# GATB/dsk

Measured on AMD Instinct MI355X. Metric: distinct k-mers counted/sec (whole node), k=31, higher is better.
Workload: dtype u64

## Files before the change

dsk_amd/csrc/dskgpu.hip:

```cpp
#include <algorithm>
#include <cstdio>
#include <cstring>
#include <cstdlib>
#include <cmath>
#include <string>
#include <vector>

#include <thread>
#include <system_error>
#include "engine.h"
#include "kernels.h"
#include "superkmer.h"
#include "rawparse.h"

#include <rocprim/device/device_radix_sort.hpp>

#define DSKGPU_VERSION "dskgpu 0.1 (gfx950)"

namespace {

thread_local std::string g_create_err;

__global__ __launch_bounds__(1024) void k_place_probe(unsigned long long* __restrict__ out, unsigned long long n) {
    const unsigned long long per_block = n / gridDim.x, per_stream = per_block / 512;
// ... 59 lines not shown
__global__ __launch_bounds__(256) void k_setup_pass(u32* __restrict__ sc, ScalarSet h, u64* __restrict__ ghist, u32 nh, u64* __restrict__ gstats, u32 nstats,
                                                    u32* __restrict__ zero, u64 nzero) {
    const u32 t = blockIdx.x * 256 + threadIdx.x;
    if (t < SC_COUNT) sc[t] = h.v[t];
    if (t < nstats) gstats[t] = 0ull;
    for (u32 i = t; i < nh; i += gridDim.x * 256) ghist[i] = 0ull;
    for (u64 i = t; i < nzero; i += (u64)gridDim.x * 256) zero[i] = 0u;
}
}

namespace {

#define LAND_BYTES (64u << 10)
void* landing(dskgpu_ctx* ctx, size_t bytes) {
    if (bytes > LAND_BYTES) return nullptr;
    if (!ctx->land && hipHostMalloc(reinterpret_cast<void**>(&ctx->land), LAND_BYTES, hipHostMallocDefault) != hipSuccess) { ctx->land = nullptr; (void)hipGetLastError(); }
    return ctx->land;
}

bool sentinel_is_a_kmer(int W, unsigned k) {
    u64 v[4] = {0, 0, 0, 0};
    if (W == 1) v[0] = kunmix(~0ull);
    else if (W == 2) { KN<2> x; x.w[0] = x.w[1] = ~0ull; kunmixN(x); v[0] = x.w[0]; v[1] = x.w[1]; }
    else { KN<4> x; for (int i = 0; i < 4; ++i) x.w[i] = ~0ull; kunmixN(x); for (int i = 0; i < 4; ++i) v[i] = x.w[i]; }
    auto base = [&](const u64* a, unsigned i) { return (unsigned)((a[i >> 5] >> (2 * (i & 31))) & 3u); };
    for (unsigned i = k; i < 128; ++i) if (base(v, i)) return false;
    u64 r[4] = {0, 0, 0, 0};
    for (unsigned i = 0; i < k; ++i) { const unsigned c = base(v, i) ^ 2u, j = k - 1 - i; r[j >> 5] |= (u64)c << (2 * (j & 31)); }
    for (int x = 3; x >= 0; --x) if (v[x] != r[x]) return v[x] < r[x];
    return true;
}


int run_encode(dskgpu_ctx* ctx, const uint8_t* d_bytes, u64 n, u64* nwords_out) {
    const u64 nwords = (n + 31) / 32;
    ctx->enc_fresh = false;
    CK(ctx->packed.ensure((nwords + 1) * 8));
    CK(ctx->inval.ensure((nwords + 1) * 4));
    if (const int rc = encode_into(ctx, d_bytes, n, ctx->packed.as<u64>(), ctx->inval.as<u32>())) return rc;
    *nwords_out = nwords;
    return DSKGPU_OK;
}

int encode_current(dskgpu_ctx* ctx, u64* nwords_out) {
    if (ctx->enc_keep) { *nwords_out = (ctx->n_bytes + 31) / 32; ctx->enc_fresh = false; return DSKGPU_OK; }
    if (!ctx->d_reads && ctx->n_bytes) return fail(ctx, DSKGPU_E_STATE, "the reads were released (dskgpu_encode_reads) and their 2-bit form has been overwritten: set the reads again");
    return run_encode(ctx, ctx->d_reads, ctx->n_bytes, nwords_out);
}

}

int encode_into(dskgpu_ctx* ctx, const uint8_t* d_bytes, u64 n, u64* packed, u32* inval) {
    const u64 nwords = (n + 31) / 32;
    if (!nwords) return DSKGPU_OK;
    const u64 nb = (nwords + 255) / 256;
    const unsigned grid = (unsigned)std::min<u64>(nb, (u64)ctx->num_cu * 16);
    if ((reinterpret_cast<uintptr_t>(d_bytes) & 15) == 0)
        hipLaunchKernelGGL(k_encode<true>, dim3(grid), dim3(256), 0, ctx->stream, d_bytes, n, packed, inval, nwords);
    else
        hipLaunchKernelGGL(k_encode<false>, dim3(grid), dim3(256), 0, ctx->stream, d_bytes, n, packed, inval, nwords);
    CKL("k_encode");
    return DSKGPU_OK;
}

int run_scan(dskgpu_ctx* ctx, u32* a, const u32* d_len, u64 max_len) {
    const u64 nb = std::max<u64>(1, (max_len + SCAN_BLK - 1) / SCAN_BLK);
    CK(ctx->sums.ensure((nb + 1) * 4));
    hipLaunchKernelGGL(k_scan_reduce, dim3((unsigned)nb), dim3(SCAN_NT), 0, ctx->stream, a, d_len, ctx->sums.as<u32>());
    hipLaunchKernelGGL(k_scan_sums, dim3(1), dim3(1024), 0, ctx->stream, ctx->sums.as<u32>(), d_len, a);
    hipLaunchKernelGGL(k_scan_apply, dim3((unsigned)nb), dim3(SCAN_NT), 0, ctx->stream, a, d_len, ctx->sums.as<u32>());
    CKL("k_scan");
    return DSKGPU_OK;
}

int allow_big_lds(dskgpu_ctx* ctx, const void* fn, int bytes) {
    for (const void* f : ctx->big_lds_fns) if (f == fn) return DSKGPU_OK;
    CK(hipFuncSetAttribute(fn, hipFuncAttributeMaxDynamicSharedMemorySize, bytes));
    ctx->big_lds_fns.push_back(fn);
    return DSKGPU_OK;
}

namespace {

size_t scatter_lds(int W, u32 P, bool opt = false) { return (size_t)SC_NT * (16 / W) * 8 * W + (size_t)P * (opt ? 20 : 16) + 4 + 17 * 4 + 16 + (opt ? 8 + L0_MAX_PASSES * 8 : 0); }

template <int W, int SRC, int MODE>
int launch_hist_m(dskgpu_ctx* ctx, const typename KeyT<W>::T* keys, const ChunkDesc* descs, const u32* d_nch,
                  u64 max_chunks, u32* matrix, DigitSpec ds, u32 P) {
    const unsigned grid = (unsigned)std::max<u64>(1, std::min<u64>(max_chunks, (u64)ctx->num_cu));
    hipLaunchKernelGGL((k_hist<W, SRC, MODE>), dim3(grid), dim3(SC_NT), 0, ctx->stream, ctx->packed.as<u64>(),
                       ctx->inval.as<u32>(), keys, descs, d_nch, matrix, (int)ctx->cfg.kmer_size, ds, P);
    CKL("k_hist");
    return DSKGPU_OK;
// ... 1029 lines not shown
    CK(ctx->l0buf.ensure(tot * sp.R * 8 + 64));
    CK(ctx->sk_lay.ensure(SK_MAX_OWNERS * 12));
    CK(hipMemcpyAsync(ctx->sk_lay.p, obase, sizeof obase, hipMemcpyHostToDevice, ctx->stream));
    CK(hipMemcpyAsync(ctx->sk_lay.as<u64>() + SK_MAX_OWNERS, osl, sizeof osl, hipMemcpyHostToDevice, ctx->stream));
    sp.olo = olo; sp.ohi = ohi; sp.obase = ctx->sk_lay.as<unsigned long long>(); sp.oslice = reinterpret_cast<const u32*>(ctx->sk_lay.as<u64>() + SK_MAX_OWNERS);
    sp.c0 = 0; sp.c0g = 0; sp.clen = (u32)rl.nch; sp.rbase = 0; sp.slice = 0;
    u32* sc = ctx->scalars.as<u32>();
    CK(hipMemsetAsync(ctx->sk_sent.p, 0, SK_MAX_OWNERS * 8, ctx->stream));
    CK(hipMemsetAsync(sc + SC_OVF1, 0, 4, ctx->stream));
#define SK_CALL(K_, M_) hipLaunchKernelGGL((k_sk_scatter<true, K_, M_>), dim3(sp.nchunks), dim3(SK_NT), 0, ctx->stream, ctx->packed.as<u64>(), ctx->inval.as<u32>(), sp, \
                                          (const unsigned long long*)nullptr, ctx->l0buf.as<u64>(), sc + SC_OVF1, ctx->sk_sent.as<unsigned long long>())
    SK_DISPATCH(ctx, sp, SK_CALL);
#undef SK_CALL
    CKL("k_sk_scatter(passes)");
    ctx->mark("level0");
    CK(hipMemcpyAsync(&ctx->h_ovf1, sc + SC_OVF1, 4, hipMemcpyDeviceToHost, ctx->stream));
    CK(hipMemcpyAsync(ctx->h_sk_sent, ctx->sk_sent.p, SK_MAX_OWNERS * 8, hipMemcpyDeviceToHost, ctx->stream));
    CK(hipStreamSynchronize(ctx->stream));
    if (ctx->tune.verbose) fprintf(stderr, "[dskgpu] level 0 (records): passes %u..%u of %u materialised, %.2f GB%s\n", olo, ohi - 1, rl.G, (double)tot * sp.R * 8e-9,
                                   ctx->h_ovf1 ? " -- a slice overflowed: starting over on the key-array path" : "");
    return ctx->h_ovf1 ? REC_L0_NO : DSKGPU_OK;
}

template <int W>
int run_pipeline(dskgpu_ctx* ctx, bool from_reads, const typename KeyT<W>::T* d_keys_in, u64 nkeys_in) {
    typedef typename KeyT<W>::T Key;
    ctx->drop_result();
    ctx->sink = dskgpu_ctx::RowSink{};
    if (from_reads) { ctx->st_names.clear(); ctx->st_ms.clear(); }
    ctx->marks.clear(); ctx->ev_used = 0;
    const u64 n_upper = from_reads ? ctx->n_bytes : nkeys_in;
    u64 nwords = 0;
    ctx->mark("start");
    if (from_reads) {
        int rc = encode_current(ctx, &nwords);
        if (rc) return rc;
        ctx->mark("encode");
    }
    CK(ctx->scalars.ensure(SC_COUNT * 4));
    CK(ctx->ghist.ensure(((size_t)ctx->cfg.histo_max + 1 + 2) * 8));
    CK(ctx->gstats.ensure(4 * 8));
    ctx->have_nvalid = false;
    if (from_reads && nwords) {
        CK(hipMemsetAsync(ctx->gstats.p, 0, 4 * 8, ctx->stream));
        hipLaunchKernelGGL(k_count_valid, dim3((unsigned)std::min<u64>((nwords + 255) / 256, (u64)ctx->num_cu * 8)), dim3(256), 0, ctx->stream,
                           ctx->inval.as<u32>(), nwords, (int)ctx->cfg.kmer_size, ctx->gstats.as<u64>() + 3);
        CKL("k_count_valid");
        {
            void* lz = landing(ctx, 8);
            CK(hipMemcpyAsync(lz ? lz : (void*)&ctx->h_nvalid, ctx->gstats.as<u64>() + 3, 8, hipMemcpyDeviceToHost, ctx->stream));
            CK(hipStreamSynchronize(ctx->stream));
            if (lz) std::memcpy(&ctx->h_nvalid, lz, 8);
        }
        ctx->have_nvalid = true;
    }
    const u64 max_keys = ctx->max_keys_per_pass ? ctx->max_keys_per_pass : 0xD0000000ull;
    const u64 n_keys = (from_reads && ctx->have_nvalid) ? std::max<u64>(1, ctx->h_nvalid) : n_upper;
    u64 pass_keys = max_keys;
    if (W == 1 && from_reads && ctx->have_nvalid && n_keys > max_keys && !ctx->max_keys_per_pass && !ctx->tune.no_level0)
        pass_keys = ctx->tune.mp_pass_mkeys ? (u64)ctx->tune.mp_pass_mkeys * 1000000ull : 1000000000ull;
    const u64 hard_max = W == 2 && !ctx->max_keys_per_pass ? std::min<u64>(max_keys, 2400000000ull) : max_keys;
    u32 npass = (u32)std::max<u64>(1, (n_keys + pass_keys - 1) / pass_keys);
    bool rec_l0 = W <= 2 && from_reads && ctx->have_nvalid && ctx->sk_mode && ctx->cfg.world_size == 1 && !ctx->tune.no_level0 && !ctx->tune.l0_keys && !ctx->rec_l0_off &&
                  (npass > 1 || n_keys > hard_max);
    RecL0 rl;
    struct SenderStateGuard {
        dskgpu_ctx* c; SkParams sp; std::vector<uint8_t> table; bool armed = false;
        ~SenderStateGuard() { if (armed) { c->sk_sp = sp; c->h_table.swap(table); c->table_dirty = true; c->sk_prepared = false; c->enc_fresh = false; } }
    } sender_guard{ctx, ctx->sk_sp, ctx->h_table};
    if (rec_l0) {
        sender_guard.armed = true;
        u64 want = ctx->max_keys_per_pass ? max_keys : ctx->tune.mp_pass_mkeys ? (u64)ctx->tune.mp_pass_mkeys * 1000000ull : (W == 1 ? 1200000000ull : 1000000000ull);
        u64 G = (n_keys + want - 1) / want;
        if (G < 2) G = 2;
        if (G > SK_MAX_OWNERS) G = SK_MAX_OWNERS;
        if (n_keys / G + n_keys / G / 7 > hard_max && !ctx->max_keys_per_pass) rec_l0 = false;
        else {
            const int rc = rec_l0_prepare(ctx, nwords, (u32)G, &rl);
            if (rc == REC_L0_NO) rec_l0 = false; else if (rc) return rc;
            else npass = (u32)G;
// ... 1143 lines not shown
    if (abundance) CK(hipMemcpy(abundance, ctx->res_ab + b, n * 4, hipMemcpyDeviceToHost));
    return DSKGPU_OK;
}

int dskgpu_result_device(const dskgpu_ctx* ctx, const void** d_kmers, const void** d_abundance, uint64_t* n_rows) {
    if (!ctx) return DSKGPU_E_ARG;
    if (!ctx->have_result) return DSKGPU_E_STATE;
    if (d_kmers) *d_kmers = ctx->res_w[0];
    if (d_abundance) *d_abundance = ctx->res_ab;
    if (n_rows) *n_rows = ctx->n_rows;
    return DSKGPU_OK;
}

int dskgpu_stage_times(const dskgpu_ctx* ctx, const char** names, float* ms, int cap) {
    if (!ctx) return DSKGPU_E_ARG;
    const int n = (int)ctx->st_names.size();
    for (int i = 0; i < n && i < cap; ++i) { if (names) names[i] = ctx->st_names[i]; if (ms) ms[i] = ctx->st_ms[i]; }
    return n;
}

int dskgpu_k_encode(dskgpu_ctx* ctx, const void* d_bytes, uint64_t nbytes, void* d_packed, void* d_invalid) {
    if (!ctx || !d_packed || !d_invalid) return DSKGPU_E_ARG;
    CK(hipSetDevice(ctx->cfg.device));
    u64 nwords = 0;
    if (ctx->enc_keep) { ctx->enc_keep = false; }
    int rc = run_encode(ctx, static_cast<const uint8_t*>(d_bytes), nbytes, &nwords);
    if (rc) return rc;
    CK(hipMemcpyAsync(d_packed, ctx->packed.p, nwords * 8, hipMemcpyDeviceToDevice, ctx->stream));
    CK(hipMemcpyAsync(d_invalid, ctx->inval.p, nwords * 4, hipMemcpyDeviceToDevice, ctx->stream));
    CK(hipStreamSynchronize(ctx->stream));
    return DSKGPU_OK;
}

int dskgpu_k_enumerate(dskgpu_ctx* ctx, const void* d_bytes, uint64_t nbytes, void* d_kmers, void* d_valid) {
    if (!ctx || !d_kmers || !d_valid) return DSKGPU_E_ARG;
    CK(hipSetDevice(ctx->cfg.device));
    u64 nwords = 0;
    if (ctx->enc_keep) { ctx->enc_keep = false; }
    int rc = run_encode(ctx, static_cast<const uint8_t*>(d_bytes), nbytes, &nwords);
    if (rc) return rc;
    if (nwords) {
        const unsigned grid = (unsigned)((nwords * 2 + 255) / 256);
        if (ctx->W == 1)
            hipLaunchKernelGGL(k_enumerate<1>, dim3(grid), dim3(256), 0, ctx->stream, ctx->packed.as<u64>(), ctx->inval.as<u32>(),
                               nwords, (u64)nbytes, (int)ctx->cfg.kmer_size, static_cast<u64*>(d_kmers), static_cast<uint8_t*>(d_valid), 1);
        else if (ctx->W == 2)
            hipLaunchKernelGGL(k_enumerate<2>, dim3(grid), dim3(256), 0, ctx->stream, ctx->packed.as<u64>(), ctx->inval.as<u32>(),
                               nwords, (u64)nbytes, (int)ctx->cfg.kmer_size, static_cast<u64*>(d_kmers), static_cast<uint8_t*>(d_valid), ctx->words_out);
        else
            hipLaunchKernelGGL(k_enumerate<4>, dim3(grid), dim3(256), 0, ctx->stream, ctx->packed.as<u64>(), ctx->inval.as<u32>(),
                               nwords, (u64)nbytes, (int)ctx->cfg.kmer_size, static_cast<u64*>(d_kmers), static_cast<uint8_t*>(d_valid), ctx->words_out);
        CKL("k_enumerate");
    }
    CK(hipStreamSynchronize(ctx->stream));
    return DSKGPU_OK;
}

int dskgpu_k_minimizers(dskgpu_ctx* ctx, const void* d_bytes, uint64_t nbytes, void* d_minim, void* d_valid) {
    if (!ctx || !d_minim || !d_valid) return DSKGPU_E_ARG;
    const int m = (int)ctx->cfg.minimizer_size, k = (int)ctx->cfg.kmer_size;
    if (m < 1 || m > 16 || m > k) return fail(ctx, DSKGPU_E_ARG, "minimizer_size must be in 1..16 and <= kmer_size");
    CK(hipSetDevice(ctx->cfg.device));
    u64 nwords = 0;
    if (ctx->enc_keep) { ctx->enc_keep = false; }
    int rc = run_encode(ctx, static_cast<const uint8_t*>(d_bytes), nbytes, &nwords);
    if (rc) return rc;
// ... 12 lines not shown
```

dsk_amd/csrc/engine.h:

```cpp
#pragma once
#include <algorithm>
#include <cstring>
#include <string>
#include <vector>

#include "../../include/dskgpu.h"
#include "layouts.h"

hipError_t placed_malloc(void** out, size_t bytes);

struct DevBuf {
    void* p = nullptr;
    size_t cap = 0;
    hipError_t ensure(size_t bytes) {
        if (bytes <= cap) return hipSuccess;
        size_t want = ((p ? bytes + bytes / 16 : bytes) + 255) & ~size_t(255);
        if (p) { (void)hipFree(p); p = nullptr; cap = 0; }
        hipError_t e = placed_malloc(&p, want);
        if (e == hipSuccess) cap = want; else p = nullptr;
        return e;
    }
    int ensure_keep(size_t bytes, size_t keep, hipStream_t stream) {
        if (bytes <= cap) return 0;
        void* np = nullptr;
// ... 203 lines not shown
        marks.push_back({name, e});
    }
    void resolve_marks() {
        for (size_t i = 0; i + 1 < marks.size(); ++i) {
            float ms = 0; (void)hipEventElapsedTime(&ms, marks[i].ev, marks[i + 1].ev);
            size_t at = 0;
            while (at < st_names.size() && std::strcmp(st_names[at], marks[i + 1].name) != 0) ++at;
            if (at == st_names.size()) { st_names.push_back(marks[i + 1].name); st_ms.push_back(ms); } else st_ms[at] += ms;
        }
        marks.clear(); ev_used = 0;
    }
};

#define CK(expr)                                                                             \
    do {                                                                                     \
        hipError_t e_ = (expr);                                                              \
        if (e_ != hipSuccess) {                                                              \
            ctx->err = std::string(#expr) + ": " + hipGetErrorString(e_);                    \
            return (e_ == hipErrorOutOfMemory) ? DSKGPU_E_NOMEM : DSKGPU_E_DEVICE;           \
        }                                                                                    \
    } while (0)

#define CKL(what)                                                                            \
    do {                                                                                     \
        hipError_t e_ = hipGetLastError();                                                   \
        if (e_ != hipSuccess) {                                                              \
            ctx->err = std::string(what) + ": " + hipGetErrorString(e_);                     \
            return DSKGPU_E_DEVICE;                                                          \
        }                                                                                    \
    } while (0)

inline int fail(dskgpu_ctx* ctx, int code, const std::string& msg) { ctx->err = msg; return code; }

int encode_into(dskgpu_ctx* ctx, const uint8_t* d_bytes, u64 n, u64* packed, u32* inval);
int run_scan(dskgpu_ctx* ctx, u32* a, const u32* d_len, u64 max_len);
int allow_big_lds(dskgpu_ctx* ctx, const void* fn, int bytes = 160 * 1024);

int order_rows(dskgpu_ctx* ctx, u64 n, u32 npass);
u64 rs_max_rows(const dskgpu_ctx* ctx);
int sort_index_multiword(dskgpu_ctx* ctx, const u64* const* rows, u64 n, int W);
u32 part_sort_nparts(const SparseRows& rows);
int launch_part_sort(dskgpu_ctx* ctx, const SparseRows& rows, RowsOut out, u32* out_ab, u32* d_part_off, u32* d_flag, u32* nparts_out);
u32 rows_partitions(const dskgpu_ctx* ctx);
void rows_partition_range(const dskgpu_ctx* ctx, u32 p, u64* b, u64* e);

struct QTable;
int ensure_index(dskgpu_ctx* ctx);
QTable query_table(const dskgpu_ctx* ctx);
int query_ensure(dskgpu_ctx* ctx, DevBuf& b, size_t bytes, const char* what);
void query_begin(dskgpu_ctx* ctx);
int query_finish(dskgpu_ctx* ctx);
```

dsk_amd/csrc/kernels.h:

```cpp
#pragma once
#include "layouts.h"

#ifndef SC_NT
#define SC_NT 1024
#endif
template <int W> struct Tile {
    static constexpr int KPT = 16 / W;
    static constexpr int KEYS = SC_NT * KPT;
    static constexpr int WORDS = KEYS / 32;
};
#define MAX_BINS 2048


template <bool ALIGNED>
__global__ __launch_bounds__(256) void k_encode(const uint8_t* __restrict__ s, u64 n,
                                                u64* __restrict__ packed, u32* __restrict__ inval, u64 nwords) {
    const u64 stride = (u64)gridDim.x * blockDim.x;
    for (u64 w = (u64)blockIdx.x * blockDim.x + threadIdx.x; w < nwords; w += stride) {
        const u64 base = w * 32;
        u32 x[8];
        if (ALIGNED && base + 32 <= n) {
            const uint4 a = *reinterpret_cast<const uint4*>(s + base);
            const uint4 b = *reinterpret_cast<const uint4*>(s + base + 16);
            x[0] = a.x; x[1] = a.y; x[2] = a.z; x[3] = a.w; x[4] = b.x; x[5] = b.y; x[6] = b.z; x[7] = b.w;
        } else {
#pragma unroll
            for (int q = 0; q < 8; ++q) {
                u32 v = 0;
#pragma unroll
                for (int b = 0; b < 4; ++b) {
                    const u64 p = base + q * 4 + b;
                    const u32 c = p < n ? s[p] : (u32)'\n';
                    v |= c << (8 * b);
                }
                x[q] = v;
            }
        }
        u64 pk = 0; u32 iv = 0;
        constexpr u32 BASES = (1u << 1) | (1u << 3) | (1u << 7) | (1u << 20);
#pragma unroll
        for (int q = 0; q < 8; ++q) {
            const u32 xx = x[q];
            const u32 codes = ((((xx >> 1) & 0x03030303u) * 0x40100401u) >> 24);
            const u32 hi = (xx & 0xC0C0C0C0u) ^ 0x40404040u;
            u32 ok = 0;
#pragma unroll
            for (int b = 0; b < 4; ++b) ok |= ((BASES >> ((xx >> (8 * b)) & 31u)) & 1u) << (8 * b);
            const u32 hz = (((hi & 0x7F7F7F7Fu) + 0x7F7F7F7Fu) | hi) >> 7;
            const u32 good = ok & ~hz & 0x01010101u;
            const u32 bad4 = (((good ^ 0x01010101u) * 0x08040201u) >> 24) & 0xFu;
            pk |= (u64)codes << (56 - 8 * q);
            iv |= bad4 << (28 - 4 * q);
        }
        packed[w] = pk;
        inval[w] = iv;
    }
}

template <int W> struct KeyT { typedef KN<W> T; };
template <> struct KeyT<1> { typedef u64 T; };

__device__ __forceinline__ u64 digit_word(u64 h) { return h; }
template <int W> __device__ __forceinline__ u64 digit_word(const KN<W>& h) { return h.w[W - 1]; }

struct DigitSpec { u32 mode, pa, pb, world, npass, pass; };
__device__ __forceinline__ u32 key_pass(u64 w, const DigitSpec& ds) {
    const u32 frac = (((u32)(w >> 12) & 0xFFFFFu) * ds.world) & 0xFFFFFu;
    return (frac * ds.npass) >> 20;
}
template <int MODE>
__device__ __forceinline__ u32 key_digit(u64 w, const DigitSpec& ds) {
    if (MODE == 1 || MODE == 3) return __umulhi((u32)(w >> 32), ds.pa);
    if (MODE == 2) return __umulhi((u32)(w >> 32) * ds.pa, ds.pb);
    if (MODE == 4) return key_pass(w, ds) - ds.pass;
    return (((u32)(w >> 12) & 0xFFFFFu) * ds.pa) >> 20;
}
template <int MODE>
__device__ __forceinline__ bool key_in_pass(u64 w, const DigitSpec& ds) {
    if (MODE == 3) return key_pass(w, ds) == ds.pass;
    if (MODE == 4) return key_pass(w, ds) - ds.pass < ds.pa;
    return true;
}

template <int NP>
__device__ __forceinline__ u32 gen_kmers_multi(const u64* __restrict__ packed, const u32* __restrict__ inval, u64 wi, int t0, int k, K2 (&c)[NP]) {
    return gen_kmers2<NP>(packed, inval, wi, t0, k, c);
}
template <int W, int NP>
// ... 331 lines not shown
        auto rank_and_stage = [&](Key (&h)[KPT], u32 vm) {
            if constexpr (HEAVY && W <= 2) {
#pragma unroll
                for (int x = 0; x < HV_KEYS; ++x) {
                    if (x < nhk) {
                        u32 hits = 0;
#pragma unroll
                        for (int j = 0; j < KPT; ++j) hits |= keys_same(h[j], hvk[x]) ? (1u << j) : 0u;
                        hits &= vm;
                        hc[x] += (u32)__popc(hits);
                        vm &= ~hits;
                    }
                }
            }
            u32 rk[KPT];
#pragma unroll
            for (int j = 0; j < KPT; ++j) {
                u32 dj = key_digit<MODE>(digit_word(h[j]), ds);
                asm volatile("" : "+v"(dj));
                dj = ((vm & (1u << j)) && key_in_pass<MODE>(digit_word(h[j]), ds)) ? dj : P;
                rk[j] = dj << 16;
            }
#pragma unroll
            for (int j = 0; j < KPT; ++j) if ((rk[j] >> 16) < P) rk[j] |= atomicAdd(&cnt[rk[j] >> 16], 1u);
            lds_barrier();
            tile_scan<SC_NT>(cnt, off, delta, cur, (int)P, wsum, tot, OPT ? SliceGuard{o1.uslice ? nullptr : lim, o1.dump, o1.uslice, first} : SliceGuard{nullptr, 0u, 0u, 0u});
            lds_barrier();
#pragma unroll
            for (int j = 0; j < KPT; ++j) if ((rk[j] >> 16) < P) stage[off[rk[j] >> 16] + (rk[j] & 0xFFFFu)] = h[j];
            lds_barrier();
        };
        auto write_out = [&]() {
            const u32 ntile = *tot;
#pragma unroll
            for (int it = 0; it < (KPT + 3) / 4; ++it) {
                const u32 i0 = (u32)it * 4 * SC_NT;
                if constexpr (W >= 4) {
#pragma unroll
                    for (int u = 0; u < 4; ++u) {
                        const u32 i = i0 + u * SC_NT + threadIdx.x;
                        const Key kv = stage[i];
                        const u32 dg = key_digit<MODE>(digit_word(kv), ds);
                        const u32 d1 = delta[MODE == 4 ? (dg < P ? dg : 0u) : dg];
                        if (OPT) out[i < ntile ? (u64)(d1 + i) : (u64)(o1.dump + i)] = kv;
                        else if (i < ntile) out[(u64)(d1 + i)] = kv;
                    }
                    continue;
                }
                Key hk[4]; u32 dd[4];
#pragma unroll
                for (int u = 0; u < 4; ++u) hk[u] = stage[i0 + u * SC_NT + threadIdx.x];
#pragma unroll
                for (int u = 0; u < 4; ++u) {
                    const u32 dg = key_digit<MODE>(digit_word(hk[u]), ds);
                    dd[u] = delta[MODE == 4 ? (dg < P ? dg : 0u) : dg];
                }
#pragma unroll
                for (int u = 0; u < 4; ++u) {
                    const u32 i = i0 + u * SC_NT + threadIdx.x;
                    if (OPT && MODE == 4) out[i < ntile ? lob[key_digit<MODE>(digit_word(hk[u]), ds) & (L0_MAX_PASSES - 1)] + (u64)(dd[u] + i) : o1.obase0 + (u64)(o1.dump + i)] = hk[u];
                    else if (OPT) out[i < ntile ? (u64)(dd[u] + i) : (u64)(o1.dump + i)] = hk[u];
                    else if (i < ntile) out[(u64)(dd[u] + i)] = hk[u];
                }
            }
        };
        auto process = [&](Key (&h)[KPT], u32 vm) { rank_and_stage(h, vm); write_out(); };
        if (SRC == 1 && d.begin < d.end) vma = tile_keys_array<W>(keys, d.begin, d.end, ha);
        lds_barrier();
        if constexpr (SRC == 2) {
            if constexpr (W <= 2) {
                RecPre<W> pre;
                if (d.begin < d.end) rec_prefetch<W>(pre, packed, o1.R, d.begin, d.end);
                for (u64 r0 = d.begin; r0 < d.end;) {
                    u32 taken = 0;
                    vma = tile_keys_records<W>(pre, o1.R, r0, d.end, k, ha, smem, wsum, &taken);
                    rank_and_stage(ha, vma);
                    r0 += taken ? taken : 1u;
                    if (r0 < d.end) rec_prefetch<W>(pre, packed, o1.R, r0, d.end);
                    write_out();
                }
            }
        } else if constexpr (SRC == 0 && W == 1) {
            struct Raw { u64 cur, prev; u32 ic, ip; };
            const u32 wlane = threadIdx.x & (SC_NT / 2 - 1);
            const bool upper = threadIdx.x >= SC_NT / 2;
            auto load_raw = [&](u64 t0) {
                const u64 wi = t0 + wlane;
                const u64 wc = wi < d.end ? wi : d.end - 1;
                Raw r; r.cur = packed[wc]; r.prev = packed[wc ? wc - 1 : 0]; r.ic = inval[wc]; r.ip = inval[wc ? wc - 1 : 0];
                if (wc == 0) { r.prev = 0ull; r.ip = 0xFFFFFFFFu; }
                return r;
            };
            if (d.begin < d.end) {
                Raw raw = load_raw(d.begin);
// ... 1621 lines not shown
```

dsk_amd/engine.py:

```python
from __future__ import annotations

import ctypes as C
import os
from typing import List, Optional, Sequence, Tuple

import numpy as np

_HERE = os.path.dirname(os.path.abspath(__file__))


class DskGpuError(RuntimeError):
    def __init__(self, code: int, msg: str):
        super().__init__(f"dskgpu error {code}: {msg}")
        self.code = code


class _Config(C.Structure):
    _fields_ = [
        ("kmer_size", C.c_uint32),
        ("abundance_min", C.c_uint32),
        ("abundance_max", C.c_uint32),
        ("histo_max", C.c_uint32),
        ("device", C.c_int32),
        ("nb_partitions", C.c_uint32),
# ... 47 lines not shown
        ("reserved", C.c_uint64 * 4),
    ]


MG_BUCKETS = 4096
MG_SPLIT = 255


def make_table(summed_loads: np.ndarray, world_size: int) -> np.ndarray:
    loads = np.ascontiguousarray(summed_loads, dtype=np.uint64)
    assert loads.size == MG_BUCKETS
    table = np.zeros(MG_BUCKETS, dtype=np.uint8)
    load_library().dskgpu_mg_make_table(loads.ctypes.data_as(C.POINTER(C.c_uint64)), world_size, table.ctypes.data_as(C.POINTER(C.c_uint8)))
    return table


F_TIMING = 1
F_NO_SORT = 2
F_HISTO2D = 4
F_MG_EXPLICIT = 8
F_PLACE = 16
F_PARTITION_ORDER = 32
SOLIDITY = {"sum": 0, "min": 1, "max": 2, "one": 3, "all": 4, "custom": 5}

EXPORTS = [
    "dskgpu_create", "dskgpu_destroy", "dskgpu_last_error", "dskgpu_version", "dskgpu_device_count", "dskgpu_set_stream",
    "dskgpu_push_reads", "dskgpu_push_raw", "dskgpu_raw_finish", "dskgpu_stream_bytes", "dskgpu_rewind_reads", "dskgpu_reserve_reads", "dskgpu_reserve_work", "dskgpu_set_reads_device", "dskgpu_encode_reads", "dskgpu_next_bank", "dskgpu_set_banks", "dskgpu_histogram2d",
    "dskgpu_count", "dskgpu_mg_scatter", "dskgpu_mg_sample", "dskgpu_mg_make_table", "dskgpu_mg_set_table",
    "dskgpu_mg_send_capacity_words", "dskgpu_mg_count", "dskgpu_mg_sent_kmers", "dskgpu_mg_count_sized",
    "dskgpu_mg_slices_prepare", "dskgpu_mg_scatter_slice", "dskgpu_mg_slices_finish", "dskgpu_mg_count_sliced", "dskgpu_get_stats", "dskgpu_histogram",
    "dskgpu_set_row_order", "dskgpu_num_partitions", "dskgpu_partition_size", "dskgpu_partition_offsets", "dskgpu_partition_copy", "dskgpu_result_device",
    "dskgpu_stage_times", "dskgpu_query_prepare", "dskgpu_query_kmers", "dskgpu_query_reads", "dskgpu_graph_adjacency", "dskgpu_graph_neighbors",
    "dskgpu_unitigs", "dskgpu_unitigs_rows", "dskgpu_unitigs_table", "dskgpu_unitigs_stream", "dskgpu_unitig_edges", "dskgpu_unitig_edges_table",
    "dskgpu_k_encode", "dskgpu_k_enumerate", "dskgpu_k_minimizers",
    "dskgpu_group_create", "dskgpu_group_destroy", "dskgpu_group_last_error", "dskgpu_group_size", "dskgpu_group_ctx",
    "dskgpu_group_transport", "dskgpu_group_count", "dskgpu_group_exchanged_words", "dskgpu_group_sliced_steps", "dskgpu_group_histogram", "dskgpu_group_histogram2d",
    "dskgpu_group_get_stats", "dskgpu_group_num_partitions", "dskgpu_group_partition_size", "dskgpu_group_partition_copy",
]

_lib = None


SLICE_GATE = C.CFUNCTYPE(C.c_int, C.c_void_p, C.c_uint32)


def library_path() -> str:
    return os.environ.get("DSKGPU_LIB", os.path.join(_HERE, "libdskgpu.so"))


def load_library():
    global _lib
    if _lib is not None:
        return _lib
    path = library_path()
    if not os.path.exists(path):
        raise ImportError(
            f"{path} not found: build it with `python -c 'import __graft_entry__ as g; g.build()'` "
            "or `make -C dsk_amd/csrc` (there is no CPU fallback for the count path)")
    lib = C.CDLL(path)
    vp, u64, u32 = C.c_void_p, C.c_uint64, C.c_uint32
    lib.dskgpu_create.argtypes = [C.POINTER(_Config), C.POINTER(vp)]
    lib.dskgpu_create.restype = C.c_int
    lib.dskgpu_destroy.argtypes = [vp]
    lib.dskgpu_destroy.restype = None
    lib.dskgpu_last_error.argtypes = [vp]
    lib.dskgpu_last_error.restype = C.c_char_p
    lib.dskgpu_version.argtypes = []
# ... 30 lines not shown
    lib.dskgpu_histogram.argtypes = [vp, C.POINTER(u64), u32]
    lib.dskgpu_num_partitions.argtypes = [vp]
    lib.dskgpu_num_partitions.restype = u32
    lib.dskgpu_set_row_order.argtypes = [vp, C.c_int]
    lib.dskgpu_partition_size.argtypes = [vp, u32]
    lib.dskgpu_partition_offsets.argtypes = [vp, vp]
    lib.dskgpu_partition_size.restype = u64
    lib.dskgpu_partition_copy.argtypes = [vp, u32, vp, vp]
    lib.dskgpu_result_device.argtypes = [vp, C.POINTER(vp), C.POINTER(vp), C.POINTER(u64)]
    lib.dskgpu_stage_times.argtypes = [vp, C.POINTER(C.c_char_p), C.POINTER(C.c_float), C.c_int]
    lib.dskgpu_query_prepare.argtypes = [vp]
    lib.dskgpu_query_prepare.restype = C.c_int
    lib.dskgpu_query_kmers.argtypes = [vp, vp, u64, vp]
    lib.dskgpu_query_kmers.restype = C.c_int
    lib.dskgpu_query_reads.argtypes = [vp, vp, u64, vp]
    lib.dskgpu_query_reads.restype = C.c_int
    lib.dskgpu_graph_adjacency.argtypes = [vp, vp, C.POINTER(u64)]
    lib.dskgpu_graph_adjacency.restype = C.c_int
    lib.dskgpu_graph_neighbors.argtypes = [vp, vp, u64, vp]
    lib.dskgpu_graph_neighbors.restype = C.c_int
    lib.dskgpu_unitigs.argtypes = [vp, C.POINTER(_UnitigStats)]
    lib.dskgpu_unitigs.restype = C.c_int
    lib.dskgpu_unitigs_rows.argtypes = [vp, vp, vp]
    lib.dskgpu_unitigs_rows.restype = C.c_int
    lib.dskgpu_unitigs_table.argtypes = [vp, vp, vp, vp]
    lib.dskgpu_unitigs_table.restype = C.c_int
    lib.dskgpu_unitigs_stream.argtypes = [vp, vp, u64]
    lib.dskgpu_unitigs_stream.restype = C.c_int
    lib.dskgpu_unitig_edges.argtypes = [vp, C.POINTER(_UnitigEdgeStats)]
    lib.dskgpu_unitig_edges.restype = C.c_int
    lib.dskgpu_unitig_edges_table.argtypes = [vp, vp, vp, vp]
    lib.dskgpu_unitig_edges_table.restype = C.c_int
    lib.dskgpu_k_encode.argtypes = [vp, vp, u64, vp, vp]
    lib.dskgpu_k_enumerate.argtypes = [vp, vp, u64, vp, vp]
    lib.dskgpu_k_minimizers.argtypes = [vp, vp, u64, vp, vp]
    lib.dskgpu_group_create.argtypes = [C.POINTER(_Config), C.POINTER(C.c_int32), u32, C.POINTER(vp)]
    lib.dskgpu_group_destroy.argtypes = [vp]
    lib.dskgpu_group_destroy.restype = None
    lib.dskgpu_group_last_error.argtypes = [vp]
    lib.dskgpu_group_last_error.restype = C.c_char_p
    lib.dskgpu_group_size.argtypes = [vp]
    lib.dskgpu_group_size.restype = u32
    lib.dskgpu_group_ctx.argtypes = [vp, u32]
    lib.dskgpu_group_ctx.restype = vp
    lib.dskgpu_group_transport.argtypes = [vp]
    lib.dskgpu_group_transport.restype = C.c_char_p
    lib.dskgpu_group_count.argtypes = [vp]
    lib.dskgpu_group_exchanged_words.argtypes = [vp]
    lib.dskgpu_group_exchanged_words.restype = u64
    lib.dskgpu_group_sliced_steps.argtypes = [vp]
    lib.dskgpu_group_sliced_steps.restype = u32
    lib.dskgpu_group_histogram.argtypes = [vp, C.POINTER(u64), u32]
    lib.dskgpu_group_histogram2d.argtypes = [vp, C.POINTER(u64), u32]
    lib.dskgpu_group_get_stats.argtypes = [vp, C.POINTER(_Stats)]
    lib.dskgpu_group_num_partitions.argtypes = [vp]
    lib.dskgpu_group_num_partitions.restype = u32
    lib.dskgpu_group_partition_size.argtypes = [vp, u32]
    lib.dskgpu_group_partition_size.restype = u64
    lib.dskgpu_group_partition_copy.argtypes = [vp, u32, vp, vp]
    for name in EXPORTS:
        getattr(lib, name)
    _lib = lib
    return lib


def _make_config(kmer_size, abundance_min, abundance_max, histo_max, device, nb_partitions, timing, sort, world_size, rank,
# ... 364 lines not shown
        self._ck(self._lib.dskgpu_unitig_edges(self._h, C.byref(st)))
        return {name: int(getattr(st, name)) for name, _ in _UnitigEdgeStats._fields_ if name != "reserved"}

    def unitig_edges_table(self, d_offsets: int, d_targets: int, d_ends: int) -> None:
        self._ck(self._lib.dskgpu_unitig_edges_table(self._h, *(C.c_void_p(p) if p else None for p in (d_offsets, d_targets, d_ends))))

    def unitig_edges_tensor(self):
        import torch
        ne = self.unitig_edges()["n_edges"]
        n_or = 2 * self.unitigs()["n_unitigs"]
        dev = torch.device("cuda", self.device)
        off = torch.zeros(n_or + 1, dtype=torch.int64, device=dev)
        targets, ends = torch.zeros(ne, dtype=torch.int32, device=dev), torch.zeros(n_or, dtype=torch.int32, device=dev)
        torch.cuda.current_stream(dev).synchronize()
        self.unitig_edges_table(off.data_ptr(), targets.data_ptr() if ne else 0, ends.data_ptr() if n_or else 0)
        return off, targets, ends

    def write_gfa(self, path: str) -> dict:
        text = bytes(self.unitigs_stream_tensor().cpu().numpy())
        ab_sum = self.unitigs_table_tensor()[1].cpu().numpy()
        off, targets, _ = (t.cpu().numpy() for t in self.unitig_edges_tensor())
        seqs = text.decode().split("\n")[:-1]
        assert len(seqs) == len(ab_sum)
        overlap = "%dM" % (self.kmer_size - 1)
        with open(path, "w") as f:
            f.write("H\tVN:Z:1.0\n")
            for u, seq in enumerate(seqs):
                f.write("S\t%d\t%s\tLN:i:%d\tKC:i:%d\n" % (u, seq, len(seq), int(ab_sum[u])))
            for U in range(2 * len(seqs)):
                for V in targets[off[U]: off[U + 1]]:
                    f.write("L\t%d\t%s\t%d\t%s\t%s\n" % (U >> 1, "-" if U & 1 else "+", int(V) >> 1, "-" if int(V) & 1 else "+", overlap))
        return {"n_segments": len(seqs), "n_links": int(len(targets))}

    def k_encode(self, d_bytes: int, nbytes: int, d_packed: int, d_invalid: int) -> None:
        self._ck(self._lib.dskgpu_k_encode(self._h, C.c_void_p(d_bytes), nbytes, C.c_void_p(d_packed), C.c_void_p(d_invalid)))

    def k_enumerate(self, d_bytes: int, nbytes: int, d_kmers: int, d_valid: int) -> None:
        self._ck(self._lib.dskgpu_k_enumerate(self._h, C.c_void_p(d_bytes), nbytes, C.c_void_p(d_kmers), C.c_void_p(d_valid)))

    def k_minimizers(self, d_bytes: int, nbytes: int, d_minim: int, d_valid: int) -> None:
        self._ck(self._lib.dskgpu_k_minimizers(self._h, C.c_void_p(d_bytes), nbytes, C.c_void_p(d_minim), C.c_void_p(d_valid)))


class KmerGroup:

    def __init__(self, devices, kmer_size: int = 31, abundance_min: int = 2, abundance_max: int = 2147483647,
                 histo_max: int = 10000, nb_partitions: int = 0, timing: bool = False, sort: bool = True,
                 minimizer_size: int = 0, max_pass_mkeys: int = 0, mg_explicit: bool = False):
        self._lib = load_library()
        devices = list(devices)
        cfg = _make_config(kmer_size, abundance_min, abundance_max, histo_max, 0, nb_partitions, timing, sort, len(devices), 0,
                           minimizer_size, max_pass_mkeys, "sum", 0, False, mg_explicit)
        devs = (C.c_int32 * len(devices))(*devices)
        h = C.c_void_p()
        rc = self._lib.dskgpu_group_create(C.byref(cfg), devs, len(devices), C.byref(h))
        if rc != 0:
            raise DskGpuError(rc, self._lib.dskgpu_group_last_error(None).decode())
        self._h = h
        self.size = len(devices)
        self.kmer_size, self.histo_max = kmer_size, histo_max
        self.words = (kmer_size + 31) // 32
        self._ranks = [KmerCounter._borrowed(self._lib.dskgpu_group_ctx(self._h, r), kmer_size, histo_max, self.size, devices[r])
                       for r in range(self.size)]

    def _ck(self, rc: int) -> None:
        if rc != 0:
# ... 60 lines not shown
```

include/dskgpu.h:

```cpp
#ifndef DSKGPU_H
#define DSKGPU_H
#include <stddef.h>
#include <stdint.h>

#ifdef __cplusplus
extern "C" {
#endif

#define DSKGPU_OK 0
#define DSKGPU_E_ARG (-1)
#define DSKGPU_E_DEVICE (-2)
#define DSKGPU_E_NOMEM (-3)
#define DSKGPU_E_STATE (-4)
#define DSKGPU_E_OVERFLOW (-5)
#define DSKGPU_E_FORMAT (-6)
#define DSKGPU_NOT_RESERVED 1

typedef struct dskgpu_ctx dskgpu_ctx;

typedef struct dskgpu_config {
    uint32_t kmer_size;
    uint32_t abundance_min;
    uint32_t abundance_max;
    uint32_t histo_max;
// ... 106 lines not shown

typedef struct dskgpu_unitig_stats {
    uint64_t n_unitigs, n_cycles, n_single, max_nodes, stream_bytes, n_rounds, reserved[2];
} dskgpu_unitig_stats;
int dskgpu_unitigs(dskgpu_ctx* ctx, dskgpu_unitig_stats* stats);
int dskgpu_unitigs_rows(dskgpu_ctx* ctx, void* d_unitig, void* d_pos);
int dskgpu_unitigs_table(dskgpu_ctx* ctx, void* d_offsets, void* d_ab_sum, void* d_kind);
int dskgpu_unitigs_stream(dskgpu_ctx* ctx, void* d_bytes, uint64_t capacity);

typedef struct dskgpu_unitig_edge_stats {
    uint64_t n_edges, n_self, n_dead_ends, max_degree, reserved[4];
} dskgpu_unitig_edge_stats;
int dskgpu_unitig_edges(dskgpu_ctx* ctx, dskgpu_unitig_edge_stats* stats);
int dskgpu_unitig_edges_table(dskgpu_ctx* ctx, void* d_offsets, void* d_targets, void* d_ends);

typedef struct dskgpu_group dskgpu_group;
int  dskgpu_group_create(const dskgpu_config* cfg, const int32_t* devices, uint32_t n_ranks, dskgpu_group** out);
void dskgpu_group_destroy(dskgpu_group* g);
const char* dskgpu_group_last_error(const dskgpu_group* g);
uint32_t dskgpu_group_size(const dskgpu_group* g);
dskgpu_ctx* dskgpu_group_ctx(dskgpu_group* g, uint32_t rank);
const char* dskgpu_group_transport(const dskgpu_group* g);
int dskgpu_group_count(dskgpu_group* g);
uint64_t dskgpu_group_exchanged_words(const dskgpu_group* g);
uint32_t dskgpu_group_sliced_steps(const dskgpu_group* g);
int dskgpu_group_histogram(const dskgpu_group* g, uint64_t* out, uint32_t nbins);
int dskgpu_group_histogram2d(const dskgpu_group* g, uint64_t* out, uint32_t nrows);
int dskgpu_group_get_stats(const dskgpu_group* g, dskgpu_stats* out);
uint32_t dskgpu_group_num_partitions(const dskgpu_group* g);
uint64_t dskgpu_group_partition_size(const dskgpu_group* g, uint32_t P);
int dskgpu_group_partition_copy(const dskgpu_group* g, uint32_t P, uint64_t* kmers, uint32_t* abundance);

int dskgpu_k_encode(dskgpu_ctx* ctx, const void* d_bytes, uint64_t nbytes, void* d_packed, void* d_invalid);
int dskgpu_k_enumerate(dskgpu_ctx* ctx, const void* d_bytes, uint64_t nbytes, void* d_kmers, void* d_valid);
int dskgpu_k_minimizers(dskgpu_ctx* ctx, const void* d_bytes, uint64_t nbytes, void* d_minim, void* d_valid);

#ifdef __cplusplus
}
#endif
#endif
```

Before: 25.36 billion.

## Fuse valid k-mer window counting into the encode kernel

The encode kernel gains a counting variant that stages each block's invalid-base masks in shared memory, with a halo from the previous words, and computes the number of valid k-mer windows in the same pass. The separate k_count_valid launch and its reread of the invalid mask array are then skipped. Separately, the superkmer write-out path clamps staged indices to the last valid slot instead of sending overflow lanes to a dump region. Possible costs are extra halo re-encoding, a __syncthreads per tile, and an atomic per block. A small API to query the valid-window count is also added.

```diff
diff --git a/dsk_amd/csrc/dskgpu.hip b/dsk_amd/csrc/dskgpu.hip
--- a/dsk_amd/csrc/dskgpu.hip
+++ b/dsk_amd/csrc/dskgpu.hip
@@ -115,33 +115,40 @@
 }
 
 
-int run_encode(dskgpu_ctx* ctx, const uint8_t* d_bytes, u64 n, u64* nwords_out) {
+int run_encode(dskgpu_ctx* ctx, const uint8_t* d_bytes, u64 n, u64* nwords_out, int k = 0, u64* total = nullptr) {
     const u64 nwords = (n + 31) / 32;
     ctx->enc_fresh = false;
     CK(ctx->packed.ensure((nwords + 1) * 8));
     CK(ctx->inval.ensure((nwords + 1) * 4));
-    if (const int rc = encode_into(ctx, d_bytes, n, ctx->packed.as<u64>(), ctx->inval.as<u32>())) return rc;
+    if (const int rc = encode_into(ctx, d_bytes, n, ctx->packed.as<u64>(), ctx->inval.as<u32>(), k, total)) return rc;
     *nwords_out = nwords;
     return DSKGPU_OK;
 }
 
-int encode_current(dskgpu_ctx* ctx, u64* nwords_out) {
+int encode_current(dskgpu_ctx* ctx, u64* nwords_out, int k = 0, u64* total = nullptr, bool* counted = nullptr) {
+    if (counted) *counted = false;
     if (ctx->enc_keep) { *nwords_out = (ctx->n_bytes + 31) / 32; ctx->enc_fresh = false; return DSKGPU_OK; }
     if (!ctx->d_reads && ctx->n_bytes) return fail(ctx, DSKGPU_E_STATE, "the reads were released (dskgpu_encode_reads) and their 2-bit form has been overwritten: set the reads again");
-    return run_encode(ctx, ctx->d_reads, ctx->n_bytes, nwords_out);
-}
-
-}
-
-int encode_into(dskgpu_ctx* ctx, const uint8_t* d_bytes, u64 n, u64* packed, u32* inval) {
+    if (const int rc = run_encode(ctx, ctx->d_reads, ctx->n_bytes, nwords_out, k, total)) return rc;
+    if (counted) *counted = total != nullptr;
+    return DSKGPU_OK;
+}
+
+}
+
+int encode_into(dskgpu_ctx* ctx, const uint8_t* d_bytes, u64 n, u64* packed, u32* inval, int k, u64* total) {
     const u64 nwords = (n + 31) / 32;
     if (!nwords) return DSKGPU_OK;
     const u64 nb = (nwords + 255) / 256;
     const unsigned grid = (unsigned)std::min<u64>(nb, (u64)ctx->num_cu * 16);
-    if ((reinterpret_cast<uintptr_t>(d_bytes) & 15) == 0)
-        hipLaunchKernelGGL(k_encode<true>, dim3(grid), dim3(256), 0, ctx->stream, d_bytes, n, packed, inval, nwords);
+    const bool aligned = (reinterpret_cast<uintptr_t>(d_bytes) & 15) == 0;
+    if (total) {
+        if (aligned) hipLaunchKernelGGL((k_encode<true, true>), dim3(grid), dim3(256), 0, ctx->stream, d_bytes, n, packed, inval, nwords, k, total);
+        else hipLaunchKernelGGL((k_encode<false, true>), dim3(grid), dim3(256), 0, ctx->stream, d_bytes, n, packed, inval, nwords, k, total);
+    } else if (aligned)
+        hipLaunchKernelGGL((k_encode<true, false>), dim3(grid), dim3(256), 0, ctx->stream, d_bytes, n, packed, inval, nwords, 0, (u64*)nullptr);
     else
-        hipLaunchKernelGGL(k_encode<false>, dim3(grid), dim3(256), 0, ctx->stream, d_bytes, n, packed, inval, nwords);
+        hipLaunchKernelGGL((k_encode<false, false>), dim3(grid), dim3(256), 0, ctx->stream, d_bytes, n, packed, inval, nwords, 0, (u64*)nullptr);
     CKL("k_encode");
     return DSKGPU_OK;
 }
@@ -1237,20 +1244,23 @@
     const u64 n_upper = from_reads ? ctx->n_bytes : nkeys_in;
     u64 nwords = 0;
     ctx->mark("start");
+    CK(ctx->gstats.ensure(4 * 8));
+    bool counted = false;
     if (from_reads) {
-        int rc = encode_current(ctx, &nwords);
+        CK(hipMemsetAsync(ctx->gstats.p, 0, 4 * 8, ctx->stream));
+        int rc = encode_current(ctx, &nwords, (int)ctx->cfg.kmer_size, ctx->gstats.as<u64>() + 3, &counted);
         if (rc) return rc;
         ctx->mark("encode");
     }
     CK(ctx->scalars.ensure(SC_COUNT * 4));
     CK(ctx->ghist.ensure(((size_t)ctx->cfg.histo_max + 1 + 2) * 8));
-    CK(ctx->gstats.ensure(4 * 8));
     ctx->have_nvalid = false;
     if (from_reads && nwords) {
-        CK(hipMemsetAsync(ctx->gstats.p, 0, 4 * 8, ctx->stream));
-        hipLaunchKernelGGL(k_count_valid, dim3((unsigned)std::min<u64>((nwords + 255) / 256, (u64)ctx->num_cu * 8)), dim3(256), 0, ctx->stream,
-                           ctx->inval.as<u32>(), nwords, (int)ctx->cfg.kmer_size, ctx->gstats.as<u64>() + 3);
-        CKL("k_count_valid");
+        if (!counted) {
+            hipLaunchKernelGGL(k_count_valid, dim3((unsigned)std::min<u64>((nwords + 255) / 256, (u64)ctx->num_cu * 8)), dim3(256), 0, ctx->stream,
+                               ctx->inval.as<u32>(), nwords, (int)ctx->cfg.kmer_size, ctx->gstats.as<u64>() + 3);
+            CKL("k_count_valid");
+        }
         {
             void* lz = landing(ctx, 8);
             CK(hipMemcpyAsync(lz ? lz : (void*)&ctx->h_nvalid, ctx->gstats.as<u64>() + 3, 8, hipMemcpyDeviceToHost, ctx->stream));
@@ -2460,6 +2470,8 @@
     return DSKGPU_OK;
 }
 
+uint64_t dskgpu_valid_windows(const dskgpu_ctx* ctx) { return ctx && ctx->have_nvalid ? ctx->h_nvalid : 0; }
+
 int dskgpu_k_enumerate(dskgpu_ctx* ctx, const void* d_bytes, uint64_t nbytes, void* d_kmers, void* d_valid) {
     if (!ctx || !d_kmers || !d_valid) return DSKGPU_E_ARG;
     CK(hipSetDevice(ctx->cfg.device));
diff --git a/dsk_amd/csrc/engine.h b/dsk_amd/csrc/engine.h
--- a/dsk_amd/csrc/engine.h
+++ b/dsk_amd/csrc/engine.h
@@ -259,7 +259,7 @@
 
 inline int fail(dskgpu_ctx* ctx, int code, const std::string& msg) { ctx->err = msg; return code; }
 
-int encode_into(dskgpu_ctx* ctx, const uint8_t* d_bytes, u64 n, u64* packed, u32* inval);
+int encode_into(dskgpu_ctx* ctx, const uint8_t* d_bytes, u64 n, u64* packed, u32* inval, int k = 0, u64* total = nullptr);
 int run_scan(dskgpu_ctx* ctx, u32* a, const u32* d_len, u64 max_len);
 int allow_big_lds(dskgpu_ctx* ctx, const void* fn, int bytes = 160 * 1024);
 
diff --git a/dsk_amd/csrc/kernels.h b/dsk_amd/csrc/kernels.h
--- a/dsk_amd/csrc/kernels.h
+++ b/dsk_amd/csrc/kernels.h
@@ -12,48 +12,116 @@
 #define MAX_BINS 2048
 
 
-template <bool ALIGNED>
+template <bool ALIGNED, bool WHOLE = false>
+__device__ __forceinline__ void encode_load(const uint8_t* __restrict__ s, u64 n, u64 w, u32 (&x)[8]) {
+    const u64 base = w * 32;
+    if (ALIGNED && (WHOLE || base + 32 <= n)) {
+        const uint4 a = *reinterpret_cast<const uint4*>(s + base);
+        const uint4 b = *reinterpret_cast<const uint4*>(s + base + 16);
+        x[0] = a.x; x[1] = a.y; x[2] = a.z; x[3] = a.w; x[4] = b.x; x[5] = b.y; x[6] = b.z; x[7] = b.w;
+    } else {
+#pragma unroll
+        for (int q = 0; q < 8; ++q) {
+            u32 v = 0;
+#pragma unroll
+            for (int b = 0; b < 4; ++b) {
+                const u64 p = base + q * 4 + b;
+                const u32 c = p < n ? s[p] : (u32)'\n';
+                v |= c << (8 * b);
+            }
+            x[q] = v;
+        }
+    }
+}
+__device__ __forceinline__ void encode_bits(const u32 (&x)[8], u64& pk_out, u32& iv_out) {
+    u64 pk = 0; u32 iv = 0;
+    constexpr u32 BASES = (1u << 1) | (1u << 3) | (1u << 7) | (1u << 20);
+#pragma unroll
+    for (int q = 0; q < 8; ++q) {
+        const u32 xx = x[q];
+        const u32 codes = ((((xx >> 1) & 0x03030303u) * 0x40100401u) >> 24);
+        const u32 hi = (xx & 0xC0C0C0C0u) ^ 0x40404040u;
+        u32 ok = 0;
+#pragma unroll
+        for (int b = 0; b < 4; ++b) ok |= ((BASES >> ((xx >> (8 * b)) & 31u)) & 1u) << (8 * b);
+        const u32 hz = (((hi & 0x7F7F7F7Fu) + 0x7F7F7F7Fu) | hi) >> 7;
+        const u32 good = ok & ~hz & 0x01010101u;
+        const u32 bad4 = (((good ^ 0x01010101u) * 0x08040201u) >> 24) & 0xFu;
+        pk |= (u64)codes << (56 - 8 * q);
+        iv |= bad4 << (28 - 4 * q);
+    }
+    pk_out = pk; iv_out = iv;
+}
+__device__ __forceinline__ u32 word_valid_windows(int k, u32 ic, const u32* p) {
+    if (k <= 32) {
+        u64 bad = ((u64)p[-1] << 32) | ic;
+        int rem = k - 1;
+#pragma unroll
+        for (int st = 1; st <= 16; st <<= 1) { const int sh = rem < st ? rem : st; bad |= bad >> sh; rem -= sh; }
+        return 32u - (u32)__popc((u32)bad);
+    }
+    if (k <= 64) {
+        u64 bad_lo = ((u64)p[-1] << 32) | ic, bad_hi = p[-2];
+        int rem = k - 1;
+#pragma unroll
+        for (int st = 1; st <= 32; st <<= 1) {
+            const int sh = rem < st ? rem : st;
+            if (sh) { bad_lo |= (bad_lo >> sh) | (bad_hi << (64 - sh)); bad_hi |= bad_hi >> sh; }
+            rem -= sh;
+        }
+        return 32u - (u32)__popc((u32)bad_lo);
+    }
+    int run = 0;
+    for (int q = 1; q <= 4 && run < k; ++q) {
+        const u32 iv = p[-q];
+        if (iv == 0) run += 32; else { run += __builtin_ctz(iv); break; }
+    }
+    const int f = ic ? __clz((int)ic) : 32;
+    const int need = k - 1 - run;
+    const int good = f - (need > 0 ? need : 0);
+    return good > 0 ? (u32)good : 0u;
+}
+template <bool ALIGNED, bool COUNT = false>
 __global__ __launch_bounds__(256) void k_encode(const uint8_t* __restrict__ s, u64 n,
-                                                u64* __restrict__ packed, u32* __restrict__ inval, u64 nwords) {
+                                                u64* __restrict__ packed, u32* __restrict__ inval, u64 nwords, int k, u64* __restrict__ total) {
     const u64 stride = (u64)gridDim.x * blockDim.x;
-    for (u64 w = (u64)blockIdx.x * blockDim.x + threadIdx.x; w < nwords; w += stride) {
-        const u64 base = w * 32;
-        u32 x[8];
-        if (ALIGNED && base + 32 <= n) {
-            const uint4 a = *reinterpret_cast<const uint4*>(s + base);
-            const uint4 b = *reinterpret_cast<const uint4*>(s + base + 16);
-            x[0] = a.x; x[1] = a.y; x[2] = a.z; x[3] = a.w; x[4] = b.x; x[5] = b.y; x[6] = b.z; x[7] = b.w;
-        } else {
-#pragma unroll
-            for (int q = 0; q < 8; ++q) {
-                u32 v = 0;
-#pragma unroll
-                for (int b = 0; b < 4; ++b) {
-                    const u64 p = base + q * 4 + b;
-                    const u32 c = p < n ? s[p] : (u32)'\n';
-                    v |= c << (8 * b);
-                }
-                x[q] = v;
-            }
-        }
-        u64 pk = 0; u32 iv = 0;
-        constexpr u32 BASES = (1u << 1) | (1u << 3) | (1u << 7) | (1u << 20);
-#pragma unroll
-        for (int q = 0; q < 8; ++q) {
-            const u32 xx = x[q];
-            const u32 codes = ((((xx >> 1) & 0x03030303u) * 0x40100401u) >> 24);
-            const u32 hi = (xx & 0xC0C0C0C0u) ^ 0x40404040u;
-            u32 ok = 0;
-#pragma unroll
-            for (int b = 0; b < 4; ++b) ok |= ((BASES >> ((xx >> (8 * b)) & 31u)) & 1u) << (8 * b);
-            const u32 hz = (((hi & 0x7F7F7F7Fu) + 0x7F7F7F7Fu) | hi) >> 7;
-            const u32 good = ok & ~hz & 0x01010101u;
-            const u32 bad4 = (((good ^ 0x01010101u) * 0x08040201u) >> 24) & 0xFu;
-            pk |= (u64)codes << (56 - 8 * q);
-            iv |= bad4 << (28 - 4 * q);
-        }
-        packed[w] = pk;
-        inval[w] = iv;
+    if constexpr (!COUNT) {
+        for (u64 w = (u64)blockIdx.x * blockDim.x + threadIdx.x; w < nwords; w += stride) {
+            u32 x[8]; u64 pk; u32 iv;
+            encode_load<ALIGNED>(s, n, w, x);
+            encode_bits(x, pk, iv);
+            packed[w] = pk;
+            inval[w] = iv;
+        }
+    } else {
+        __shared__ u32 siv[2][4 + 256];
+        __shared__ u32 ws[4];
+        u32 c = 0, par = 0;
+        for (u64 wb = (u64)blockIdx.x * 256; wb < nwords; wb += stride, par ^= 1u) {
+            u32* sv = siv[par] + 4;
+            const u64 w = wb + threadIdx.x;
+            const bool halo = threadIdx.x >= 252 && wb;
+            u32 x[8], hx[8]; u64 pk; u32 iv = 0xFFFFFFFFu, hv = 0xFFFFFFFFu;
+            if (w < nwords) encode_load<ALIGNED>(s, n, w, x);
+            if (halo) encode_load<ALIGNED, true>(s, n, wb - (256u - threadIdx.x), hx);
+            if (w < nwords) {
+                encode_bits(x, pk, iv);
+                packed[w] = pk;
+                inval[w] = iv;
+            }
+            sv[threadIdx.x] = iv;
+            if (threadIdx.x >= 252) {
+                if (halo) { u64 hp; encode_bits(hx, hp, hv); }
+                sv[(int)threadIdx.x - 256] = hv;
+            }
+            __syncthreads();
+            if (w < nwords) c += word_valid_windows(k, iv, sv + threadIdx.x);
+        }
+#pragma unroll
+        for (int d = 32; d >= 1; d >>= 1) c += __shfl_down(c, d);
+        if ((threadIdx.x & 63) == 0) ws[threadIdx.x >> 6] = c;
+        __syncthreads();
+        if (threadIdx.x == 0) atomicAdd(total, (u64)ws[0] + ws[1] + ws[2] + ws[3]);
     }
 }
 
@@ -451,24 +519,27 @@
         };
         auto write_out = [&]() {
             const u32 ntile = *tot;
+            const u32 last = ntile - 1u;
+            auto slot = [&](u32 i) { return OPT ? (i < last ? i : last) : i; };
+            auto base = [&](u32 dl) { return OPT ? (ntile ? dl : o1.dump) : dl; };
 #pragma unroll
             for (int it = 0; it < (KPT + 3) / 4; ++it) {
                 const u32 i0 = (u32)it * 4 * SC_NT;
                 if constexpr (W >= 4) {
 #pragma unroll
                     for (int u = 0; u < 4; ++u) {
-                        const u32 i = i0 + u * SC_NT + threadIdx.x;
-                        const Key kv = stage[i];
+                        const u32 i = i0 + u * SC_NT + threadIdx.x, ie = slot(i);
+                        const Key kv = stage[ie];
                         const u32 dg = key_digit<MODE>(digit_word(kv), ds);
                         const u32 d1 = delta[MODE == 4 ? (dg < P ? dg : 0u) : dg];
-                        if (OPT) out[i < ntile ? (u64)(d1 + i) : (u64)(o1.dump + i)] = kv;
+                        if (OPT) out[(u64)(base(d1) + ie)] = kv;
                         else if (i < ntile) out[(u64)(d1 + i)] = kv;
                     }
                     continue;
                 }
                 Key hk[4]; u32 dd[4];
 #pragma unroll
-                for (int u = 0; u < 4; ++u) hk[u] = stage[i0 + u * SC_NT + threadIdx.x];
+                for (int u = 0; u < 4; ++u) hk[u] = stage[slot(i0 + u * SC_NT + threadIdx.x)];
 #pragma unroll
                 for (int u = 0; u < 4; ++u) {
                     const u32 dg = key_digit<MODE>(digit_word(hk[u]), ds);
@@ -476,9 +547,9 @@
                 }
 #pragma unroll
                 for (int u = 0; u < 4; ++u) {
-                    const u32 i = i0 + u * SC_NT + threadIdx.x;
-                    if (OPT && MODE == 4) out[i < ntile ? lob[key_digit<MODE>(digit_word(hk[u]), ds) & (L0_MAX_PASSES - 1)] + (u64)(dd[u] + i) : o1.obase0 + (u64)(o1.dump + i)] = hk[u];
-                    else if (OPT) out[i < ntile ? (u64)(dd[u] + i) : (u64)(o1.dump + i)] = hk[u];
+                    const u32 i = i0 + u * SC_NT + threadIdx.x, ie = slot(i);
+                    if (OPT && MODE == 4) out[(ntile ? lob[key_digit<MODE>(digit_word(hk[u]), ds) & (L0_MAX_PASSES - 1)] : o1.obase0) + (u64)(base(dd[u]) + ie)] = hk[u];
+                    else if (OPT) out[(u64)(base(dd[u]) + ie)] = hk[u];
                     else if (i < ntile) out[(u64)(dd[u] + i)] = hk[u];
                 }
             }
diff --git a/dsk_amd/engine.py b/dsk_amd/engine.py
--- a/dsk_amd/engine.py
+++ b/dsk_amd/engine.py
@@ -103,7 +103,7 @@
     "dskgpu_set_row_order", "dskgpu_num_partitions", "dskgpu_partition_size", "dskgpu_partition_offsets", "dskgpu_partition_copy", "dskgpu_result_device",
     "dskgpu_stage_times", "dskgpu_query_prepare", "dskgpu_query_kmers", "dskgpu_query_reads", "dskgpu_graph_adjacency", "dskgpu_graph_neighbors",
     "dskgpu_unitigs", "dskgpu_unitigs_rows", "dskgpu_unitigs_table", "dskgpu_unitigs_stream", "dskgpu_unitig_edges", "dskgpu_unitig_edges_table",
-    "dskgpu_k_encode", "dskgpu_k_enumerate", "dskgpu_k_minimizers",
+    "dskgpu_k_encode", "dskgpu_valid_windows", "dskgpu_k_enumerate", "dskgpu_k_minimizers",
     "dskgpu_group_create", "dskgpu_group_destroy", "dskgpu_group_last_error", "dskgpu_group_size", "dskgpu_group_ctx",
     "dskgpu_group_transport", "dskgpu_group_count", "dskgpu_group_exchanged_words", "dskgpu_group_sliced_steps", "dskgpu_group_histogram", "dskgpu_group_histogram2d",
     "dskgpu_group_get_stats", "dskgpu_group_num_partitions", "dskgpu_group_partition_size", "dskgpu_group_partition_copy",
@@ -200,6 +200,8 @@
     lib.dskgpu_unitig_edges_table.argtypes = [vp, vp, vp, vp]
     lib.dskgpu_unitig_edges_table.restype = C.c_int
     lib.dskgpu_k_encode.argtypes = [vp, vp, u64, vp, vp]
+    lib.dskgpu_valid_windows.argtypes = [vp]
+    lib.dskgpu_valid_windows.restype = u64
     lib.dskgpu_k_enumerate.argtypes = [vp, vp, u64, vp, vp]
     lib.dskgpu_k_minimizers.argtypes = [vp, vp, u64, vp, vp]
     lib.dskgpu_group_create.argtypes = [C.POINTER(_Config), C.POINTER(C.c_int32), u32, C.POINTER(vp)]
@@ -630,6 +632,9 @@
                     f.write("L\t%d\t%s\t%d\t%s\t%s\n" % (U >> 1, "-" if U & 1 else "+", int(V) >> 1, "-" if int(V) & 1 else "+", overlap))
         return {"n_segments": len(seqs), "n_links": int(len(targets))}
 
+    def valid_windows(self) -> int:
+        return int(self._lib.dskgpu_valid_windows(self._h))
+
     def k_encode(self, d_bytes: int, nbytes: int, d_packed: int, d_invalid: int) -> None:
         self._ck(self._lib.dskgpu_k_encode(self._h, C.c_void_p(d_bytes), nbytes, C.c_void_p(d_packed), C.c_void_p(d_invalid)))
 
diff --git a/include/dskgpu.h b/include/dskgpu.h
--- a/include/dskgpu.h
+++ b/include/dskgpu.h
@@ -162,6 +162,7 @@
 int dskgpu_group_partition_copy(const dskgpu_group* g, uint32_t P, uint64_t* kmers, uint32_t* abundance);
 
 int dskgpu_k_encode(dskgpu_ctx* ctx, const void* d_bytes, uint64_t nbytes, void* d_packed, void* d_invalid);
+uint64_t dskgpu_valid_windows(const dskgpu_ctx* ctx);
 int dskgpu_k_enumerate(dskgpu_ctx* ctx, const void* d_bytes, uint64_t nbytes, void* d_kmers, void* d_valid);
 int dskgpu_k_minimizers(dskgpu_ctx* ctx, const void* d_bytes, uint64_t nbytes, void* d_minim, void* d_valid);
 
```

Result: slower. 24.72 billion (-2.5%).
